# shroglck/open-pi-zero

Hardware: AMD Instinct MI355X
Metric: train samples/sec at gbsz 1024 (bf16 fwd+bwd+clip+AdamW) (higher is better)
Workload: dtype bf16; 1 GPU; Pi0 bridge training step: 256 img + 20 text + 1 proprio + 4 action tokens; model=pi0 (SigLIP-So400m/14 + Gemma-2B + 0.3B action expert), global_batch=1024, micro_batch=256, grad_accum=4, seq_len=281, parallelism=dp1

## Files before the change

### include/pz_abi.h

```cpp
#ifndef PZ_ABI_H
#define PZ_ABI_H

#include <stdint.h>

#ifdef __cplusplus
extern "C" {
#endif

#define PZ_ABI_VERSION 21

enum {
  PZ_OK = 0,
  PZ_ERR_INVALID_ARG = 1,
  PZ_ERR_LAUNCH = 2,
  PZ_ERR_UNSUPPORTED = 3,
};

enum {
  PZ_EPI_NONE = 0,
  PZ_EPI_GELU = 1,
  PZ_EPI_GEGLU = 2,
  PZ_EPI_SILU = 3,
  PZ_EPI_DGELU = 4,
  PZ_EPI_DSILU = 5,
  PZ_EPI_DGEGLU = 6,
};

typedef struct pz_gemm_args {
  int64_t M, N, K;
  const void* A; int64_t lda; int32_t a_kcontig;
  const void* B; int64_t ldb; int32_t b_kcontig;
  void* C; int64_t ldc; int32_t c_fp32;
  int64_t batch, batch_inner;
  int64_t sA_outer, sA_inner, sB_outer, sB_inner, sC_outer, sC_inner, sR_outer, sR_inner;
  int32_t epilogue;
  float alpha;
  int32_t beta_accum;
  const void* bias;
  const void* resid; int64_t ld_resid;
  void* aux; int64_t ld_aux;
  int64_t geglu_inter;
  void* workspace; int64_t ws_bytes;
  const void* norm_w; float norm_eps;
  int32_t fp8_mode; const float* a_row_scale;
} pz_gemm_args;
int pz_gemm(const pz_gemm_args* args, void* stream);
#define PZ_ABSMAX_PARTS 1024
int pz_fp8_quant_vt(const void* v, int64_t ldv, int64_t v_bstride, int64_t Z, int64_t nk, void* vt, float* vs,
                    int64_t ldt, void* stream);
int pz_fp8_quant_attn(const void* q, int64_t nqr, const void* k, int64_t nkr, const void* v, int64_t ldv,
                      int64_t v_bstride, int64_t Z, int64_t nk, void* qc, float* qs, void* kc, float* ks, void* vt,
                      float* vs, int64_t ldt, void* stream);
int pz_rmsnorm_fwd_f8(const void* x, int64_t ldx, const void* w, void* q, int64_t ldq, float* qscale, int64_t R,
                      int64_t D, float eps, void* stream);
int pz_layernorm_fwd_f8(const void* x, int64_t ldx, const void* w, const void* b, void* q, int64_t ldq, float* qscale,
                        int64_t R, int64_t D, float eps, void* stream);
int pz_fp8_quant_rows(const void* x, int64_t ldx, void* q, int64_t ldq, float* row_scale, int64_t R, int64_t D,
                      void* stream);
int pz_fp8_quant_tensor(const void* x, int64_t n, void* q, float inv_scale, void* stream);
int pz_fp8_absmax(const void* x, int64_t n, float* parts, void* stream);
const char* pz_gemm_kernel_name(const pz_gemm_args* args);

typedef struct pz_small_gemm_args {
  int64_t M, N, K;
  const void* A; int64_t sAm, sAk;
  const void* B; int64_t sBk, sBn;
  void* C; int64_t ldc;
  const void* bias;
  float alpha;
  int32_t beta;
} pz_small_gemm_args;
int pz_gemm_small(const pz_small_gemm_args* args, void* stream);

int pz_rmsnorm_fwd(const void* x, int64_t ldx, const void* w, void* y, int64_t ldy, float* rstd,
                   int64_t R, int64_t D, float eps, void* stream);
int pz_rmsnorm_bwd(const void* dy, int64_t lddy, const void* x, int64_t ldx, const void* w,
                   const float* rstd, const void* dres, void* dx, int64_t lddx, float* dw_part,
                   int64_t R, int64_t D, void* stream);
int pz_layernorm_fwd(const void* x, int64_t ldx, const void* w, const void* b, void* y, int64_t ldy,
// ... 174 lines not shown
```

### open-pi-zero_amd/csrc/pz_gemm.hip

```cpp
#include <stdarg.h>
#include <stdio.h>
#include <stdlib.h>
#include <string.h>

#include <type_traits>

#include "pz_gemm_epi.h"

namespace {

constexpr int BM = 128, BN = 128, BK = 64, NT = 256;
constexpr int TILE_BYTES = 128 * 64 * 2;


__device__ __forceinline__ i32x8 cat_f8(const bf16x8& lo, const bf16x8& hi) {
  const u32x4 a = __builtin_bit_cast(u32x4, lo), b = __builtin_bit_cast(u32x4, hi);
  return i32x8{(int)a[0], (int)a[1], (int)a[2], (int)a[3], (int)b[0], (int)b[1], (int)b[2], (int)b[3]};
}

__device__ __forceinline__ int sw_tr(int k) { return ((k & 3) | (((k >> 3) & 1) << 2)) << 2; }

template <bool KC>
__device__ __forceinline__ void g2r(u32x4 (&r)[4], const bf16_t* __restrict__ base, int64_t ld,
                                    int64_t row0, int64_t R, int64_t k0, int64_t K,
// ... 690 lines not shown
#pragma unroll
    for (int i = 0; i < CPB; ++i) {
      const int c = threadIdx.x + (half * CPB + i) * NT2;
      const int im = c >> 12, row = (c >> 4) & 255, ch = c & 15;
      const int col = im * 128 + ch * 8;
      iv[i] = *reinterpret_cast<const u32x4*>(smem + im * 65536 + row * 256 + ((ch ^ (row & 15)) << 4));
      a0[i] = X0 ? *reinterpret_cast<const u32x4*>(X0 + row * ld0 + col) : u32x4{0u, 0u, 0u, 0u};
      a1[i] = X1 ? *reinterpret_cast<const u32x4*>(X1 + row * ld1 + col) : u32x4{0u, 0u, 0u, 0u};
    }
#pragma unroll
    for (int i = 0; i < CPB; ++i) {
      const int c = threadIdx.x + (half * CPB + i) * NT2;
      const int im = c >> 12, row = (c >> 4) & 255, ch = c & 15;
      const int col = im * 128 + ch * 8;
      float v[8], x0[8], x1[8];
      unpack8(iv[i], v);
      unpack8(a0[i], x0);
      unpack8(a1[i], x1);
      bf16_t* Cp = C + row * p.ldc + col;
      if (FM == FM_DGEGLU) {
        float dg[8], du[8];
#pragma unroll
        for (int e = 0; e < 8; ++e) {
          float gl_, gr_;
          gelu_tanh_both(x0[e], gl_, gr_);
          dg[e] = v[e] * x1[e] * gr_;
          du[e] = v[e] * gl_;
        }
        st16(Cp, pack8v(dg), p.nt_store);
        st16(Cp + p.geglu_I, pack8v(du), p.nt_store);
      } else if (FM == FM_DACT) {
#pragma unroll
        for (int e = 0; e < 8; ++e) v[e] *= gelu ? gelu_tanh_grad(x0[e]) : silu_grad(x0[e]);
        st16(Cp, pack8v(v), p.nt_store);
      } else {
        if (act) {
          if (p.aux) st16(p.aux + (m0 + row) * p.ld_aux + n0 + col, iv[i], p.nt_aux);
#pragma unroll
          for (int e = 0; e < 8; ++e) v[e] = gelu ? gelu_tanh(v[e]) : silu(v[e]);
        }
#pragma unroll
        for (int e = 0; e < 8; ++e) v[e] += x1[e] + x0[e];
        st16(Cp, pack8v(v), p.nt_store);
      }
    }
  }
}

__device__ __forceinline__ void epi8p_rope(const GemmP& p, int64_t m0, int64_t n0, int wr, int wc, int lane,
                                           const f32x4 (&acc)[8][4], char* smem) {
  const int g4 = 4 * (lane >> 4), rl = lane & 15;
  char* img = smem + (wc >> 1) * 65536;
#pragma unroll
  for (int rb = 0; rb < 8; ++rb)
#pragma unroll
    for (int cb = 0; cb < 4; ++cb) {
      float v[4];
#pragma unroll
      for (int r = 0; r < 4; ++r) v[r] = acc[rb][cb][r] * p.alpha;
      img_put(img, wr * 128 + rb * 16 + rl, (wc & 1) * 64 + cb * 16 + g4, u32x2{pack2bf(v[0], v[1]), pack2bf(v[2], v[3])});
    }
  lds_sync();
  const int64_t h = n0 >> 8;
#pragma unroll 2
  for (int it = 0; it < 8; ++it) {
    const int c = threadIdx.x + it * NT2, row = c >> 4, ch = c & 15;
    const int64_t m = m0 + row;
    if (m >= p.M) continue;
    const int off = (ch ^ (row & 15)) << 4;
    const u32x4 w1 = *reinterpret_cast<const u32x4*>(smem + row * 256 + off);
    const u32x4 w2 = *reinterpret_cast<const u32x4*>(smem + 65536 + row * 256 + off);
    const int64_t b = m / p.rT, t = m - b * p.rT;
    if (h == p.rnh + 1) {
      bf16_t* dv = p.rv + (b * p.rLk + p.rkoff + t) * 256 + ch * 8;
      *reinterpret_cast<u32x4*>(dv) = w1;
      *reinterpret_cast<u32x4*>(dv + 128) = w2;
      continue;
// ... 1266 lines not shown

template <bool AKC, bool BKC, bool GEGLU, bool KTAIL>
static int launch8p_k(const GemmP& p, int64_t batch, hipStream_t st) {
  const int smem = 2 * P8_BUF;
  const bool kh = use_khalf(AKC, BKC, p.M, p.N, p.K);
  auto kern = kh ? gemm8k_kernel<AKC, BKC, GEGLU, KTAIL> : gemm8p_kernel<AKC, BKC, GEGLU, KTAIL>;
  static bool attr_set[2] = {false, false};
  if (!attr_set[kh]) {
    hipFuncSetAttribute((const void*)kern, hipFuncAttributeMaxDynamicSharedMemorySize, smem);
    attr_set[kh] = true;
  }
  const int T = p.tiles_m * p.tiles_n;
  const int units = p.tail_s ? p.dp_tiles + (T - p.dp_tiles) * p.tail_s : T;
  hipLaunchKernelGGL(kern, dim3(units, (unsigned)batch), dim3(NT2), smem, st, p);
  PZ_CHECK_LAUNCH();
  if (p.tail_s) {
    launch_tail<GEGLU>(p, T, st);
    PZ_CHECK_LAUNCH();
  }
  return PZ_OK;
}

template <bool AKC, bool BKC, bool GEGLU>
static int launch8p(const GemmP& p, int64_t batch, hipStream_t st) {
  if (p.K % 64 != 0) return launch8p_k<AKC, BKC, GEGLU, true>(p, batch, st);
  return launch8p_k<AKC, BKC, GEGLU, false>(p, batch, st);
}

static bool use_8phase() {
  const char* e = getenv("PZ_GEMM_BIG");
  return !(e && strcmp(e, "2stage") == 0);
}

extern "C" int pz_gemm(const pz_gemm_args* a, void* stream) {
  PZ_CHECK_ARG(a != nullptr, "pz_gemm: null args");
  PZ_CHECK_ARG(a->M > 0 && a->N > 0 && a->K > 0, "pz_gemm: bad dims M=%lld N=%lld K=%lld",
               (long long)a->M, (long long)a->N, (long long)a->K);
  PZ_CHECK_ARG(a->A && a->B && a->C, "pz_gemm: null operand");
  PZ_CHECK_ARG(a->batch >= 1 && a->batch_inner >= 1 && a->batch % a->batch_inner == 0,
               "pz_gemm: bad batch %lld/%lld", (long long)a->batch, (long long)a->batch_inner);
  PZ_CHECK_ARG(PZ_ALIGNED(a->A, 16) && PZ_ALIGNED(a->B, 16), "pz_gemm: A/B must be 16-byte aligned");
  PZ_CHECK_ARG(a->lda % 8 == 0 && a->ldb % 8 == 0, "pz_gemm: lda/ldb must be multiples of 8");
  PZ_CHECK_ARG(a->ldc % 4 == 0 && PZ_ALIGNED(a->C, 8), "pz_gemm: ldc %% 4 and C 8-byte alignment");
  PZ_CHECK_ARG(a->sA_outer % 8 == 0 && a->sA_inner % 8 == 0 && a->sB_outer % 8 == 0 &&
                   a->sB_inner % 8 == 0 && a->sC_outer % 4 == 0 && a->sC_inner % 4 == 0,
               "pz_gemm: batch strides must keep 16-byte alignment");
  if (a->a_kcontig) PZ_CHECK_ARG(a->K % 8 == 0, "pz_gemm: k-contiguous A needs K %% 8 == 0");
  else PZ_CHECK_ARG(a->M % 8 == 0, "pz_gemm: k-strided A needs M %% 8 == 0");
  if (a->b_kcontig) PZ_CHECK_ARG(a->K % 8 == 0, "pz_gemm: k-contiguous B needs K %% 8 == 0");
  else PZ_CHECK_ARG(a->N % 8 == 0, "pz_gemm: k-strided B needs N %% 8 == 0");
  const bool geglu = a->epilogue == PZ_EPI_GEGLU;
  if (geglu) {
    PZ_CHECK_ARG(a->b_kcontig && a->geglu_inter > 0 && a->N == 2 * a->geglu_inter && a->batch == 1 &&
                     !a->beta_accum && !a->resid && !a->bias && !a->c_fp32 && a->geglu_inter % 4 == 0,
                 "pz_gemm: GEGLU needs k-contiguous B = [gate; up] (N = 2I), no batch/bias/resid");
  }
  if (a->epilogue == PZ_EPI_GELU || a->epilogue == PZ_EPI_SILU)
    PZ_CHECK_ARG(a->batch == 1, "pz_gemm: activation epilogue is unbatched");
  PZ_CHECK_ARG(a->epilogue >= PZ_EPI_NONE && a->epilogue <= PZ_EPI_DGEGLU, "pz_gemm: unknown epilogue %d",
               (int)a->epilogue);
  PZ_CHECK_ARG(!(a->c_fp32 && a->beta_accum && a->resid), "pz_gemm: fp32 beta accumulation takes no resid");
  if (a->epilogue >= PZ_EPI_DGELU) {
    PZ_CHECK_ARG(a->batch == 1 && a->aux && !a->bias && !a->resid && !a->beta_accum && !a->c_fp32,
                 "pz_gemm: backward epilogues read aux, write bf16 C, unbatched, no bias/resid/beta");
    if (a->epilogue == PZ_EPI_DGEGLU)
      PZ_CHECK_ARG(a->geglu_inter == a->N && a->ldc >= 2 * a->N && a->ld_aux >= 2 * a->N,
// ... 25 lines not shown

  GemmP p;
  memset(&p, 0, sizeof(p));
  p.A = (const bf16_t*)a->A;
  p.B = (const bf16_t*)a->B;
  p.C = a->C;
  p.bias = (const bf16_t*)a->bias;
  p.resid = (const bf16_t*)a->resid;
  p.aux = (bf16_t*)a->aux;
  p.M = a->M; p.N = a->N; p.K = a->K;
  p.lda = a->lda; p.ldb = a->ldb; p.ldc = a->ldc;
  p.ld_resid = a->ld_resid; p.ld_aux = a->ld_aux; p.geglu_I = a->geglu_inter;
  p.batch_inner = a->batch_inner;
  p.sAo = a->sA_outer; p.sAi = a->sA_inner;
  p.sBo = a->sB_outer; p.sBi = a->sB_inner;
  p.sCo = a->sC_outer; p.sCi = a->sC_inner;
  p.sRo = a->sR_outer; p.sRi = a->sR_inner;
  p.epi = a->epilogue;
  p.c_fp32 = a->c_fp32;
  p.beta = a->beta_accum;
  p.alpha = a->alpha;
  p.nw = (const bf16_t*)a->norm_w;
  p.neps = a->norm_eps;
  p.rs = a->fp8_mode == 1 ? a->a_row_scale : nullptr;
  {
    const char* e = getenv("PZ_GEMM_DBG");
    p.dbg = e ? atoi(e) : 0;
    e = getenv("PZ_GEMM_NT");
    p.nt_store = e ? atoi(e) : 0;
    e = getenv("PZ_GEMM_NT_AUX");
    p.nt_aux = p.nt_store || (e && atoi(e) != 0);
  }
  hipStream_t st = (hipStream_t)stream;

  const Plan pl = make_plan(a);
  {
    const char* e = getenv("PZ_GEMM_GROUP");
    if (e && atoi(e) >= 1 && atoi(e) <= 64) p.group = atoi(e);
    else p.group = (a->K >= 16384 && pl.tiles_n <= 8) || a->epilogue == PZ_EPI_DGEGLU ? 2 : 8;
  }
  if (pl.kind == PATH_GEMV) return pz_gemv_launch(a, st);
  if (a->norm_w)
    PZ_CHECK_ARG((pl.kind == PATH_SKINNY || pl.kind == PATH_SKINNY64) && PZ_ALIGNED(a->norm_w, 16),
                 "pz_gemm: fused RMSNorm needs the few-row paths (M <= 64, k-contiguous A/B, K %% 32 == 0 "
                 "(M <= 16) or K %% 64 == 0) and a 16-byte aligned weight");
  if (pl.kind == PATH_SKINNY64) {
    p.tiles_n = (int)pl.tiles_n;
    if (pl.ksplit > 0) {
      p.ws = (float*)a->workspace;
      p.ksplit = pl.ksplit;
      p.ldw = pl.ldw;
      p.sk_tk = sk64_fits(pl, a) ? 0 : -1;
    }
    return pz_sk64_launch(p, pl.skinny_w, pl.skinny_nc, pl.skinny_mb, a->fp8_mode == 2, pl.tiles_n, st);
  }
  if (a->fp8_mode == 1 && pl.kind == PATH_ROWS) {
    p.tiles_m = (int)pl.tiles_m;
    p.tiles_n = (int)pl.tiles_n;
    PZ_CHECK_ARG(PZ_ALIGNED(a->A, 16) && PZ_ALIGNED(a->B, 16), "pz_gemm: W8A8 rows need 16-byte aligned codes");
    return pz_rows_launch(p, pl.rows_w, pl.rows_tnb, false, 2, st);
  }
  if (a->fp8_mode == 1) {
    p.tiles_m = (int)pl.tiles_m;
    p.tiles_n = (int)pl.tiles_n;
    PZ_CHECK_ARG(pl.tiles_m * pl.tiles_n < (1LL << 31), "pz_gemm: grid too large");
    if (pl.tail_s) {
// ... 4 lines not shown
    }
    return geglu ? launch8p_f8<true>(p, st) : launch8p_f8<false>(p, st);
  }
  if (pl.kind == PATH_SKINNY) {
    PZ_CHECK_ARG(a->batch < 65536, "pz_gemm: batch too large");
    if (pl.skinny_w == 16) return launch_skinny<16>(p, pl.skinny_nc, pl.tiles_n, a->batch, st);
    if (pl.skinny_w == 8) return launch_skinny<8>(p, pl.skinny_nc, pl.tiles_n, a->batch, st);
    return launch_skinny<4>(p, pl.skinny_nc, pl.tiles_n, a->batch, st);
  }
  p.tiles_m = (int)pl.tiles_m;
  p.tiles_n = (int)pl.tiles_n;
  PZ_CHECK_ARG(pl.tiles_m * pl.tiles_n < (1LL << 31) && a->batch < 65536, "pz_gemm: grid too large");
  if (pl.kind == PATH_ROWS)
    return pz_rows_launch(p, pl.rows_w, pl.rows_tnb, pl.geglu, pl.rows_f8, st);
  if (pl.kind == PATH_TALL) {
    if (pl.splits > 1) {
      p.ws = (float*)a->workspace;
      p.ksplit = pl.ksplit;
      p.ldw = pl.ldw;
    }
    return pz_tall_launch(p, pl.tall_mi, geglu, pl.bkc, pl.splits > 1 ? pl.splits : 1, st);
  }
  if (pl.kind == PATH_256 && use_8phase()) {
    if (pl.tail_s) {
      p.ws = (float*)a->workspace;
      p.dp_tiles = pl.dp_tiles;
      p.tail_s = pl.tail_s;
      p.tail_kt = pl.tail_kt;
    }
    if (geglu) {
      if (a->a_kcontig) return launch8p<true, true, true>(p, a->batch, st);
      return launch8p<false, true, true>(p, a->batch, st);
    }
    if (a->a_kcontig && a->b_kcontig) return launch8p<true, true, false>(p, a->batch, st);
    if (a->a_kcontig && !a->b_kcontig) return launch8p<true, false, false>(p, a->batch, st);
    if (!a->a_kcontig && a->b_kcontig) return launch8p<false, true, false>(p, a->batch, st);
    return launch8p<false, false, false>(p, a->batch, st);
  }
  if (pl.kind == PATH_256) {
    if (geglu) {
      if (a->a_kcontig) return launch256<true, true, true>(p, a->batch, st);
      return launch256<false, true, true>(p, a->batch, st);
    }
    if (a->a_kcontig && a->b_kcontig) return launch256<true, true, false>(p, a->batch, st);
    if (a->a_kcontig && !a->b_kcontig) return launch256<true, false, false>(p, a->batch, st);
    if (!a->a_kcontig && a->b_kcontig) return launch256<false, true, false>(p, a->batch, st);
    return launch256<false, false, false>(p, a->batch, st);
  }
  if (pl.kind == PATH_SPLIT) {
    p.ws = (float*)a->workspace;
    p.ksplit = pl.ksplit;
    p.ldw = pl.ldw;
  }
  if (geglu) {
    if (pl.tag) return launch_tile_any<true, true, 4, 1>(p, pl, a->batch, st);
    if (a->a_kcontig) return launch_tile_any<true, true, 4, 0>(p, pl, a->batch, st);
    return launch_tile_any<false, true, 4, 0>(p, pl, a->batch, st);
  }
  if (a->a_kcontig && a->b_kcontig) return launch_tile_any<true, true, 2, 0>(p, pl, a->batch, st);
  if (a->a_kcontig && !a->b_kcontig) return launch_tile_any<true, false, 2, 0>(p, pl, a->batch, st);
  if (!a->a_kcontig && a->b_kcontig) return launch_tile_any<false, true, 2, 0>(p, pl, a->batch, st);
  return launch_tile_any<false, false, 2, 0>(p, pl, a->batch, st);
}

extern "C" int pz_gemm_qkv_rope(const pz_qkv_rope_args* a, void* stream) {
  PZ_CHECK_ARG(a && a->x && a->W && a->pos && a->cs && a->k_out && a->v_out && a->M > 0 && a->K > 0,
               "gemm_qkv_rope: bad args");
  PZ_CHECK_ARG(a->nh >= 1 && a->N == (a->nh + 2) * a->hd && a->T > 0 && a->M % a->T == 0,
               "gemm_qkv_rope: N = (nh + 2) * hd, M %% T == 0");
  if (a->hd != BT || !a->q_out) return PZ_ERR_UNSUPPORTED;
// ... 79 lines not shown
```

### open-pi-zero_amd/csrc/pz_gemm_epi.h

```cpp
#pragma once

#include <type_traits>

#include "pz_common.h"

struct GemmP {
  const bf16_t* A;
  const bf16_t* B;
  void* C;
  const bf16_t* bias;
  const bf16_t* resid;
  bf16_t* aux;
  int64_t M, N, K, lda, ldb, ldc, ld_resid, ld_aux, geglu_I;
  int64_t batch_inner, sAo, sAi, sBo, sBi, sCo, sCi, sRo, sRi;
  int tiles_m, tiles_n, epi, c_fp32, beta;
  float alpha;
  float* ws;
  int64_t ksplit, ldw;
  int sk_tk;
  int batch_xcd;
  int dp_tiles, tail_s, tail_kt;
  const bf16_t* nw;
  float neps;
  const float* rs;
  int dbg;
  const int64_t* rpos;
  const float* rcs;
  bf16_t *rq, *rk, *rv;
  int64_t rT, rnh, rLq, rqoff, rLk, rkoff;
  int nt_store;
  int nt_aux;
  int group;
};

namespace {

__device__ __forceinline__ void tile_coords(int bid, int nwg, int tiles_m, int tiles_n, int& tm, int& tn,
                                            int GROUP = 8) {
  const int xcd = bid & 7, local = bid >> 3;
  const int q = nwg >> 3, r = nwg & 7;
  const int wg = (xcd < r ? xcd * (q + 1) : r * (q + 1) + (xcd - r) * q) + local;
  GROUP = GROUP >= 1 ? GROUP : 8;
  const int per_group = GROUP * tiles_n;
  const int g = wg / per_group;
  const int first_m = g * GROUP;
  const int gsize = min(tiles_m - first_m, GROUP);
  const int in = wg - g * per_group;
  tm = first_m + in % gsize;
  tn = in / gsize;
}

struct Side {
  u32x4 w;
};

__device__ __forceinline__ u32x2 ld4bf(const bf16_t* X, bool full, int64_t n, int64_t N) {
  if (full) return *reinterpret_cast<const u32x2*>(X);
  unsigned h[4];
#pragma unroll
  for (int r = 0; r < 4; ++r) h[r] = n + r < N ? (unsigned)X[r] : 0u;
  return u32x2{h[0] | (h[1] << 16), h[2] | (h[3] << 16)};
}
__device__ __forceinline__ void unpack4(u32x2 w, float (&o)[4]) {
  o[0] = __uint_as_float(w[0] << 16); o[1] = __uint_as_float(w[0] & 0xffff0000u);
  o[2] = __uint_as_float(w[1] << 16); o[3] = __uint_as_float(w[1] & 0xffff0000u);
// ... 135 lines not shown
  Side s;
  epi_load4<EM>(p, cofs, rofs, m, n, s);
  epi_store4<EM>(p, cofs, rofs, m, n, acc, s, epi_load_bias(p, n));
}

__device__ __forceinline__ void store_out4_rt(const GemmP& p, int64_t cofs, int64_t rofs, int64_t m, int64_t n,
                                              const f32x4& acc) {
  if (m >= p.M || n >= p.N) return;
  const bool full = n + 4 <= p.N;
  float v[4];
#pragma unroll
  for (int r = 0; r < 4; ++r) v[r] = acc[r] * p.alpha;
  if (p.epi == PZ_EPI_DGEGLU) {
    float g[4], u[4], dg[4], du[4];
    const bf16_t* X = p.aux + m * p.ld_aux + n;
    unpack4(ld4bf(X, full, n, p.N), g);
    unpack4(ld4bf(X + p.geglu_I, full, n, p.N), u);
#pragma unroll
    for (int r = 0; r < 4; ++r) {
      float gl_, gr_;
      gelu_tanh_both(g[r], gl_, gr_);
      dg[r] = v[r] * u[r] * gr_;
      du[r] = v[r] * gl_;
    }
    bf16_t* Cp = reinterpret_cast<bf16_t*>(p.C) + cofs + m * p.ldc + n;
    store4(Cp, full, n, p.N, dg);
    store4(Cp + p.geglu_I, full, n, p.N, du);
    return;
  }
  if (p.epi == PZ_EPI_DGELU || p.epi == PZ_EPI_DSILU) {
    float x[4];
    unpack4(ld4bf(p.aux + m * p.ld_aux + n, full, n, p.N), x);
#pragma unroll
    for (int r = 0; r < 4; ++r) v[r] *= p.epi == PZ_EPI_DGELU ? gelu_tanh_grad(x[r]) : silu_grad(x[r]);
  }
  if (p.bias) {
    float b[4];
    unpack4(ld4bf(p.bias + n, full, n, p.N), b);
#pragma unroll
    for (int r = 0; r < 4; ++r) v[r] += b[r];
  }
  if (p.epi == PZ_EPI_GELU || p.epi == PZ_EPI_SILU) {
    if (p.aux) store4(p.aux + m * p.ld_aux + n, full, n, p.N, v);
#pragma unroll
    for (int r = 0; r < 4; ++r) v[r] = p.epi == PZ_EPI_GELU ? gelu_tanh(v[r]) : silu(v[r]);
  }
  if (p.resid) {
    float x[4];
    unpack4(ld4bf(p.resid + rofs + m * p.ld_resid + n, full, n, p.N), x);
#pragma unroll
    for (int r = 0; r < 4; ++r) v[r] += x[r];
  }
  if (p.c_fp32) {
    float* Cp = reinterpret_cast<float*>(p.C) + cofs + m * p.ldc + n;
#pragma unroll
    for (int r = 0; r < 4; ++r)
      if (full || n + r < p.N) Cp[r] = p.beta ? Cp[r] + v[r] : v[r];
  } else {
    bf16_t* Cp = reinterpret_cast<bf16_t*>(p.C) + cofs + m * p.ldc + n;
    if (p.beta) {
      float o[4];
      unpack4(ld4bf(Cp, full, n, p.N), o);
#pragma unroll
      for (int r = 0; r < 4; ++r) v[r] += o[r];
    }
    store4(Cp, full, n, p.N, v);
  }
// ... 46 lines not shown
```

### open-pi-zero_amd/pizero_native/_lib.py

```python

from __future__ import annotations

import ctypes as C
import os

_HERE = os.path.dirname(os.path.dirname(os.path.abspath(__file__)))
LIB_PATH = os.path.join(_HERE, "libpizero_hip.so")
if os.environ.get("PZ_LIB_PATH"):
    LIB_PATH = os.path.join(_HERE, os.path.basename(os.environ["PZ_LIB_PATH"]))
    import sys as _sys

    print(f"[pizero_native] PZ_LIB_PATH override: loading {LIB_PATH} instead of the default libpizero_hip.so",
          file=_sys.stderr, flush=True)

ABI_VERSION = 21
PZ_EPI_NONE, PZ_EPI_GELU, PZ_EPI_GEGLU, PZ_EPI_SILU = 0, 1, 2, 3
PZ_EPI_DGELU, PZ_EPI_DSILU, PZ_EPI_DGEGLU = 4, 5, 6
PZ_SUMSQ_PARTS = 2048

i64, i32, f32, vp = C.c_int64, C.c_int32, C.c_float, C.c_void_p
fp = C.POINTER(C.c_float)


class GemmArgs(C.Structure):
    _fields_ = [
        ("M", i64), ("N", i64), ("K", i64),
        ("A", vp), ("lda", i64), ("a_kcontig", i32),
        ("B", vp), ("ldb", i64), ("b_kcontig", i32),
        ("C", vp), ("ldc", i64), ("c_fp32", i32),
        ("batch", i64), ("batch_inner", i64),
        ("sA_outer", i64), ("sA_inner", i64), ("sB_outer", i64), ("sB_inner", i64),
        ("sC_outer", i64), ("sC_inner", i64), ("sR_outer", i64), ("sR_inner", i64),
        ("epilogue", i32), ("alpha", f32), ("beta_accum", i32),
        ("bias", vp), ("resid", vp), ("ld_resid", i64), ("aux", vp), ("ld_aux", i64),
        ("geglu_inter", i64),
        ("workspace", vp), ("ws_bytes", i64),
        ("norm_w", vp), ("norm_eps", f32),
        ("fp8_mode", i32), ("a_row_scale", vp),
    ]


class SmallGemmArgs(C.Structure):
    _fields_ = [
        ("M", i64), ("N", i64), ("K", i64),
        ("A", vp), ("sAm", i64), ("sAk", i64),
        ("B", vp), ("sBk", i64), ("sBn", i64),
        ("C", vp), ("ldc", i64), ("bias", vp), ("alpha", f32), ("beta", i32),
    ]


class SoftmaxArgs(C.Structure):
    _fields_ = [
        ("S", vp), ("lds", i64), ("P", vp), ("ldp", i64), ("tcap", vp),
        ("R", i64), ("N", i64), ("scale", f32), ("cap", f32), ("mask_mode", i32),
        ("rows_per_batch", i64), ("heads", i64), ("qoff", i64),
        ("cnt", vp), ("prefix", i64), ("cond", i64),
        ("mask", vp), ("ldm", i64), ("mask_bstride", i64),
    ]


class FlashArgs(C.Structure):
    _fields_ = [
        ("Z", i64), ("H", i64), ("nq", i64), ("nk", i64), ("head_dim", i64),
        ("q", vp), ("ldq", i64), ("q_bstride", i64), ("q_hstride", i64),
        ("k", vp), ("ldk", i64), ("k_bstride", i64), ("k_hstride", i64),
        ("v", vp), ("ldv", i64), ("v_bstride", i64), ("v_hstride", i64),
        ("n_groups", i32),
        ("g_row0", i64 * 3), ("g_o", vp * 3), ("g_bstride", i64 * 3), ("g_ld", i64 * 3),
        ("o_hstride", i64),
        ("lse", vp),
        ("scale", f32), ("cap", f32),
# ... 20 lines not shown
class QkvRopeArgs(C.Structure):
    _fields_ = [
        ("x", vp), ("ldx", i64), ("W", vp), ("ldw", i64), ("M", i64), ("N", i64), ("K", i64),
        ("norm_w", vp), ("norm_eps", f32), ("pos", vp), ("cs", vp), ("q_out", vp), ("k_out", vp), ("v_out", vp),
        ("T", i64), ("nh", i64), ("hd", i64), ("Lq", i64), ("qoff", i64), ("Lk", i64), ("koff", i64),
        ("w_fp8", i32), ("w_scale", f32),
    ]


class ReduceSeg(C.Structure):
    _fields_ = [("part", vp), ("P", i64), ("D", i64), ("out", vp), ("beta", i32)]


class DecodeAttnArgs(C.Structure):
    _fields_ = [
        ("q", vp), ("ldq", i64), ("Lq", i64), ("qoff", i64), ("k", vp), ("v", vp), ("k_bstride", i64),
        ("v_bstride", i64), ("o", vp), ("ldo", i64), ("B", i64), ("nh", i64), ("T", i64), ("nk", i64),
        ("head_dim", i64), ("scale", f32), ("cap", f32), ("cnt", vp), ("prefix", i64), ("cond", i64),
        ("qtok0", i64), ("ws", vp), ("ws_bytes", i64),
    ]


SIGNATURES = {
    "pz_gemm": [C.POINTER(GemmArgs), vp],
    "pz_fp8_quant_rows": [vp, i64, vp, i64, vp, i64, i64, vp],
    "pz_fp8_quant_tensor": [vp, i64, vp, f32, vp],
    "pz_fp8_quant_vt": [vp, i64, i64, i64, i64, vp, vp, i64, vp],
    "pz_rmsnorm_fwd_f8": [vp, i64, vp, vp, i64, vp, i64, i64, f32, vp],
    "pz_layernorm_fwd_f8": [vp, i64, vp, vp, vp, i64, vp, i64, i64, f32, vp],
    "pz_fp8_quant_attn": [vp, i64, vp, i64, vp, i64, i64, i64, i64, vp, vp, vp, vp, vp, vp, i64, vp],
    "pz_flash_fwd_f8": [C.POINTER(FlashArgs), vp, vp, vp, vp, i64, vp, vp, i64, vp],
    "pz_fp8_absmax": [vp, i64, vp, vp],
    "pz_gemm_kernel_name": [C.POINTER(GemmArgs)],
    "pz_gemm_small": [C.POINTER(SmallGemmArgs), vp],
    "pz_rmsnorm_fwd": [vp, i64, vp, vp, i64, vp, i64, i64, f32, vp],
    "pz_rmsnorm_bwd": [vp, i64, vp, i64, vp, vp, vp, vp, i64, vp, i64, i64, vp],
    "pz_layernorm_fwd": [vp, i64, vp, vp, vp, i64, vp, vp, i64, i64, f32, vp],
    "pz_layernorm_bwd": [vp, i64, vp, i64, vp, vp, vp, vp, vp, i64, vp, vp, i64, i64, vp, vp],
    "pz_act_bwd_colsum": [vp, i64, vp, i64, vp, i64, i64, i32, vp, i64, vp, i32, vp],
    "pz_reduce_parts_multi": [vp, i32, vp],
    "pz_norm_rows_per_part": [],
    "pz_reduce_parts": [vp, i64, i64, vp, i32, vp],
    "pz_colsum": [vp, i64, i64, i64, vp, i32, vp, vp],
    "pz_batch_sum": [vp, i64, i64, i64, vp, i32, vp],
    "pz_rope_table": [vp, i64, i64, f32, vp],
    "pz_qkv_rope_split": [vp, vp, vp, vp, vp, vp, i64, i64, i64, i64, i64, i64, i64, i64, i64, vp],
    "pz_qkv_rope_split_bwd": [vp, vp, vp, vp, vp, vp, i64, i64, i64, i64, i64, i64, i64, i64, i64, vp],
    "pz_gemv_qkv_rope": [C.POINTER(QkvRopeArgs), vp],
    "pz_gemm_qkv_rope": [C.POINTER(QkvRopeArgs), vp],
    "pz_decode_attn": [C.POINTER(DecodeAttnArgs), vp],
    "pz_decode_attn_ws_bytes": [i64, i64, i64],
    "pz_attn_softmax": [C.POINTER(SoftmaxArgs), vp],
    "pz_attn_softmax_bwd": [vp, vp, i64, vp, vp, i64, i64, i64, f32, f32, vp],
    "pz_flash_fwd": [C.POINTER(FlashArgs), vp],
    "pz_flash_fwd_probs": [C.POINTER(FlashArgs), vp, vp, i64, vp],
    "pz_flash_bwd_ds": [C.POINTER(FlashArgs), vp, vp, vp, i64, vp],
    "pz_flash_bwd_prep": [C.POINTER(FlashArgs), vp],
    "pz_flash_bwd": [C.POINTER(FlashArgs), vp],
    "pz_patchify": [vp, vp, i64, i64, i64, i64, i64, vp],
    "pz_embed_merge": [vp, vp, i64, vp, vp, i64, i64, i64, i64, i64, i64, f32, f32, vp],
    "pz_embed_merge_bwd": [vp, vp, vp, i64, i64, i64, i64, i64, f32, vp],
    "pz_time_embed": [vp, vp, i64, i64, f32, i32, vp],
    "pz_concat_time": [vp, vp, vp, i64, i64, i64, vp],
    "pz_split_time_grad": [vp, vp, i64, i64, vp],
    "pz_flow_psi": [vp, vp, vp, vp, i64, i64, f32, vp],
    "pz_flow_loss": [vp, i64, i64, vp, vp, vp, vp, vp, i64, i64, i64, f32, vp],
# ... 18 lines not shown
    "pz_debug_poison_lds": [C.c_uint32, vp],
    "pz_debug_spin": [i64, i64, vp],
    "pz_last_error": [],
    "pz_abi_version": [],
}
_RESTYPE = {"pz_last_error": C.c_char_p, "pz_gemm_kernel_name": C.c_char_p, "pz_norm_rows_per_part": i64,
            "pz_decode_attn_ws_bytes": i64}

_lib = None


class NativeError(RuntimeError):
    pass


def lib():
    global _lib
    if _lib is None:
        if not os.path.exists(LIB_PATH):
            raise NativeError(
                f"{LIB_PATH} not found: build it with `python open-pi-zero_amd/build_native.py` "
                "(or __graft_entry__.build()); the Pi0 path has no CPU/eager fallback")
        L = C.CDLL(LIB_PATH)
        for name, argt in SIGNATURES.items():
            fn = getattr(L, name)
            fn.argtypes = argt
            fn.restype = _RESTYPE.get(name, C.c_int)
        if L.pz_abi_version() != ABI_VERSION:
            raise NativeError(f"{LIB_PATH}: ABI version {L.pz_abi_version()} != {ABI_VERSION}; rebuild it")
        _lib = L
    return _lib


_NO_LAUNCH = {"pz_last_error", "pz_abi_version", "pz_gemm_kernel_name", "pz_norm_rows_per_part",
              "pz_decode_attn_ws_bytes", "pz_debug_poison_lds"}
_POISON_LDS = [0xFFFFFFFF if os.environ.get("PZ_POISON_LDS", "0") == "1" else None]


_RECENT = [[] if os.environ.get("PZ_CHECK_FINITE", "0") == "1" else None]


def recent_launches(clear=True):
    r = _RECENT[0] or []
    if clear and _RECENT[0] is not None:
        _RECENT[0] = []
    return r


def set_poison_lds(word):
    _POISON_LDS[0] = None if word is None else int(word) & 0xFFFFFFFF


def call(name, *args):
    if _POISON_LDS[0] is not None and name not in _NO_LAUNCH:
        rc = lib().pz_debug_poison_lds(_POISON_LDS[0], args[-1])
        if rc != 0:
            raise NativeError(f"pz_debug_poison_lds failed (rc={rc}): {lib().pz_last_error().decode(errors='replace')}")
    if _RECENT[0] is not None:
        _RECENT[0].append(name)
    rc = getattr(lib(), name)(*args)
    if rc != 0:
        msg = lib().pz_last_error().decode(errors="replace")
        raise NativeError(f"{name} failed (rc={rc}): {msg}")
    return rc
```

### open-pi-zero_amd/pizero_native/engine.py

```python

from __future__ import annotations

import contextlib
import math
import os
import weakref
from dataclasses import dataclass

import torch

from . import ops
from .ops import PZ_EPI_DGEGLU, PZ_EPI_DGELU, PZ_EPI_GEGLU, PZ_EPI_GELU, PZ_EPI_NONE, PZ_EPI_SILU

BF16 = torch.bfloat16
F32 = torch.float32


def _cfg(cfg, key, default=None):
    from src.utils.config import cfg_get

    return cfg_get(cfg, key, default)


@dataclass
# ... 163 lines not shown
            for i, n in enumerate(w):
                if eng.rg(n):
                    ops.linear_wgrad(dm[:, i * self.D:(i + 1) * self.D], cond, eng.gw(n), beta=beta)
        if all(eng.rg(n) for n in b):
            ops.colsum(dm[:, : len(b) * self.D], eng.ar.grad_span(b[0], b[-1]), ws, beta=beta)
        else:
            for i, n in enumerate(b):
                if eng.rg(n):
                    ops.colsum(dm[:, i * self.D:(i + 1) * self.D], eng.gw(n), ws, beta=beta)


class Group:

    def __init__(self, name, prefix, mixtures, T, joint_off, hidden, inter, theta, skip_last, pos_key):
        self.name, self.prefix, self.mixtures = name, prefix, mixtures
        self.T, self.off, self.hid, self.inter, self.theta = T, joint_off, hidden, inter, theta
        self.skip_last = skip_last
        self.pos_key = pos_key


class Engine:
    def __init__(self, model):
        self.m = model
        self.d = Dims.from_cfg(model.cfg)
        self._tables = {}
        self._ws = {}
        self._jkv_holder = None
        ja = os.environ.get("PZ_JOINT_ATTN", "probs")
        self.joint_flash = ja == "flash"
        self.joint_probs = ja == "probs"
        self.joint_ds = os.environ.get("PZ_JOINT_DS", "1") == "1"
        self.joint_ds_dq = os.environ.get("PZ_JOINT_DS_DQ", "1") == "1"
        self.infer_flash = os.environ.get("PZ_INFER_ATTN", "flash") == "flash"
        self.split_dact = os.environ.get("PZ_SPLIT_DACT", "1") == "1"
        self.split_dgeglu = os.environ.get("PZ_SPLIT_DGEGLU", "0") == "1"
        self.fuse_qkv_rope = os.environ.get("PZ_FUSE_QKV_ROPE", "1") == "1" and self.d.hd == 256
        self.expert_stream = os.environ.get("PZ_EXPERT_STREAM", "1") == "1"
        self.expert_stream_fwd = os.environ.get("PZ_EXPERT_STREAM_FWD", "0") == "1"
        vI = self.d.vI
        self.sig_pitch = vI if os.environ.get("PZ_SIG_PITCH", "1") == "0" else (vI + 63) // 64 * 64
        self._side = {}
        self.check_finite = os.environ.get("PZ_CHECK_FINITE", "0") == "1"
        self.f8_attn = os.environ.get("PZ_FP8_ATTN", "1") == "1"
        self.f8 = None
        self.f8_version = None
        if self.d.nkv != 1:
            raise NotImplementedError("joint attention kernel path assumes MQA (num_key_value_heads=1, bridge.yaml:176)")

    def ada_slots(self, prefix):
        key = ("ada_slots", prefix)
        sl = self._tables.get(key)
        if sl is None:
            from src.model.vla.pizero import adaln_slots

            sl = self._tables[key] = adaln_slots(prefix, self.d.nL, self.d.ada)
        return sl

    def _chk(self, where, **tensors):
        if not self.check_finite:
            return
        check_finite(where, **tensors)

    @property
    def ar(self):
        return self.m._arena

    def w(self, name):
# ... 248 lines not shown
        fb = os.environ.get("PZ_FUSED_BIAS_GRAD", "1") != "0" and os.environ.get("PZ_NORM_BWD", "row")[:1] != "w"
        pd = torch.empty(P, d.vH, device=dev, dtype=F32) if fb else None
        pdn = torch.empty(P, d.vH, device=dev, dtype=F32) if fb else None
        pd2 = torch.empty(P, d.vH, device=dev, dtype=F32) if fb else None
        multi = os.environ.get("PZ_REDUCE_MULTI", "1") != "0"
        pw2 = torch.empty(P, d.vH, device=dev, dtype=F32) if multi else pw
        pb2 = torch.empty(P, d.vH, device=dev, dtype=F32) if multi else pb
        ws_act = self.colsum_ws_rows(1024, d.vI) if fb else None
        nm = "multi_modal_projector.linear."
        if self.rg(nm + "weight"):
            ops.linear_wgrad(dimg, sv["y"], self.gw(nm + "weight"), beta=beta)
        if self.rg(nm + "bias"):
            ops.colsum(dimg, self.gw(nm + "bias"), ws, beta=beta)
        dy = torch.empty(M, d.vH, device=dev, dtype=BF16)
        ops.linear_dgrad(dimg, self.w(nm + "weight"), dy)
        dx = torch.empty_like(dy)
        ops.layernorm_bwd(dy, sv["x_last"], self.w(vt + "post_layernorm.weight"), sv["mu"], sv["r"], dx,
                          dw_part=pw, db_part=pb, dx_part=pd)
        self._norm_grads(vt + "post_layernorm.", pw, pb, beta)
        nh, hd = d.vheads, d.vH // d.vheads
        Np = d.img_tok
        W3 = 3 * d.vH
        dg = self._sig_rows(M, dev)
        delta = torch.empty(B * nh, Np, device=dev, dtype=F32)
        dqkv = torch.empty(M, W3, device=dev, dtype=BF16)
        dh = torch.empty(M, d.vH, device=dev, dtype=BF16)
        dxm = torch.empty(M, d.vH, device=dev, dtype=BF16)
        dO = torch.empty(M, d.vH, device=dev, dtype=BF16)
        for i in reversed(range(d.vL)):
            p = f"{vt}encoder.layers.{i}."
            st = sv["layers"][i]
            red = [] if multi else None
            fc1b = self.rg(p + "mlp.fc1.bias")
            if self.split_dact:
                ops.linear_dgrad(dx, self.w(p + "mlp.fc2.weight"), dg)
                if fb and fc1b:
                    ops.act_bwd_colsum(dg, st["a1"], dg, PZ_EPI_GELU, ws_act, self.gw(p + "mlp.fc1.bias"), beta=beta)
                else:
                    ops.act_bwd(dg, st["a1"], dg, None, PZ_EPI_GELU)
            else:
                ops.linear_dgrad(dx, self.w(p + "mlp.fc2.weight"), dg, epi=PZ_EPI_DGELU, aux=st["a1"])
            if self.rg(p + "mlp.fc2.weight"):
                ops.linear_wgrad(dx, st["g1"], self.gw(p + "mlp.fc2.weight"), beta=beta)
            st["g1"] = None
            if self.rg(p + "mlp.fc2.bias"):
                if fb:
                    self._reduce(red, pd, self.gw(p + "mlp.fc2.bias"), beta)
                else:
                    ops.colsum(dx, self.gw(p + "mlp.fc2.bias"), ws, beta=beta)
            if self.rg(p + "mlp.fc1.weight"):
                ops.linear_wgrad(dg, st["h2"], self.gw(p + "mlp.fc1.weight"), beta=beta)
            if fc1b and not (fb and self.split_dact):
                ops.colsum(dg, self.gw(p + "mlp.fc1.bias"), ws, beta=beta)
            ops.linear_dgrad(dg, self.w(p + "mlp.fc1.weight"), dh)
            ops.layernorm_bwd(dh, st["xm"], self.w(p + "layer_norm2.weight"), st["mu2"], st["r2"], dxm, dres=dx,
                              dw_part=pw2, db_part=pb2, dx_part=pd2)
            self._norm_grads(p + "layer_norm2.", pw2, pb2, beta, red)
            if self.rg(p + "self_attn.out_proj.weight"):
                ops.linear_wgrad(dxm, st["O"], self.gw(p + "self_attn.out_proj.weight"), beta=beta)
            if self.rg(p + "self_attn.out_proj.bias"):
                if fb:
                    self._reduce(red, pd2, self.gw(p + "self_attn.out_proj.bias"), beta)
                else:
                    ops.colsum(dxm, self.gw(p + "self_attn.out_proj.bias"), ws, beta=beta)
            ops.linear_dgrad(dxm, self.w(p + "self_attn.out_proj.weight"), dO)
            ops.flash_bwd(ops.siglip_flash_args(st["qkv"], st["O"], st["lse"], B, nh, hd, Np, dO=dO, delta=delta,
                                                dqkv=dqkv))
            qn, vn = p + "self_attn.q_proj.", p + "self_attn.v_proj."
            if all(self.rg(p + f"self_attn.{k}_proj.weight") for k in "qkv"):
                ops.linear_wgrad(dqkv, st["h1"], self.ar.grad_span(qn + "weight", vn + "weight"), beta=beta)
            else:
                for k, c0 in (("q", 0), ("k", d.vH), ("v", 2 * d.vH)):
                    if self.rg(p + f"self_attn.{k}_proj.weight"):
                        ops.linear_wgrad(dqkv[:, c0:c0 + d.vH], st["h1"], self.gw(p + f"self_attn.{k}_proj.weight"),
                                         beta=beta)
            if all(self.rg(p + f"self_attn.{k}_proj.bias") for k in "qkv"):
                ops.colsum(dqkv, self.ar.grad_span(qn + "bias", vn + "bias"), ws, beta=beta)
            ops.linear_dgrad(dqkv, self.qkv_siglip(p), dh)
            dxn = torch.empty_like(dx)
            ops.layernorm_bwd(dh, st["x"], self.w(p + "layer_norm1.weight"), st["mu1"], st["r1"], dxn, dres=dxm,
                              dw_part=pw, db_part=pb, dx_part=pdn)
            self._norm_grads(p + "layer_norm1.", pw, pb, beta, red)
            if red:
                ops.reduce_parts_multi(red, beta=beta)
            pd, pdn = pdn, pd
# ... 1068 lines not shown
```

### open-pi-zero_amd/pizero_native/ops.py

```python

from __future__ import annotations

import ctypes as C

import torch

from ._lib import (
    PZ_EPI_DGEGLU,
    PZ_EPI_DGELU,
    PZ_EPI_DSILU,
    PZ_EPI_GEGLU,
    PZ_EPI_GELU,
    PZ_EPI_NONE,
    PZ_EPI_SILU,
    PZ_SUMSQ_PARTS,
    AdamW8Args,
    QkvRopeArgs,
    DecodeAttnArgs,
    FlashArgs,
    GemmArgs,
    SmallGemmArgs,
    NativeError,
    SoftmaxArgs,
    call,
# ... 163 lines not shown
              resid, 0 if resid is None else resid.stride(0), aux, 0 if aux is None else aux.stride(0),
              N // 2 if epi == PZ_EPI_GEGLU else 0, 1, 1, (0, 0), (0, 0), (0, 0), (0, 0), workspace(out.device),
              norm)
    a.fp8_mode = 2 if x_scale is None else 1
    a.a_row_scale = _p(x_scale)
    call("pz_gemm", C.byref(a), _st())
    return out


def rows_w8a8_ok(M, K, ncols, epi=PZ_EPI_NONE):
    import os

    if os.environ.get("PZ_ROWS_W8A8") == "0":
        return False
    return 64 < M <= 1024 and K % 128 == 0 and K <= 2048 and ncols <= 4096 and epi != PZ_EPI_GEGLU


def rows_w8a16_ok(M, K, ncols):
    import os

    if os.environ.get("PZ_GEMM_ROWS") == "0" or os.environ.get("PZ_ROWS_W8A16") == "0":
        return False
    maxm = int(os.environ.get("PZ_ROWS_MAXM", "1024"))
    return 64 < M <= maxm and K % 64 == 0 and (os.environ.get("PZ_GEMM_ROWS") == "1" or (K <= 2048 and ncols <= 4096))


def linear_dgrad(dy, W, dx, *, beta=False, resid=None, epi=PZ_EPI_NONE, aux=None):
    M, N = dy.shape
    K = W.shape[1]
    gemm(M, K, N, dy, dy.stride(0), True, W, W.stride(0), False, dx, dx.stride(0), beta=beta,
         resid=resid, ld_resid=0 if resid is None else resid.stride(0), epi=epi, aux=aux,
         ld_aux=0 if aux is None else aux.stride(0), geglu_inter=K if epi == PZ_EPI_DGEGLU else 0)
    return dx


def _split_k(M, N, K):
    tiles = ((N + 255) // 256) * ((K + 255) // 256)
    if tiles >= 160 or M < 4096 or N < 512 or K < 512 or M % 8 == 0:
        return 1
    best = 1
    for s in (2, 4, 8):
        if M % (s * 64) == 0:
            best = s
            if tiles * s >= 240:
                break
    return best


def linear_wgrad(dy, x, dW, *, beta=False):
    M, N = dy.shape
    K = x.shape[1]
    S = _split_k(M, N, K) if dW.is_contiguous() else 1
    if S == 1:
        gemm(N, K, M, dy, dy.stride(0), False, x, x.stride(0), False, dW, dW.stride(0), beta=beta)
        return dW
    Mc = M // S
    slabs = torch.empty(S, N, K, device=dW.device, dtype=torch.float32)
    gemm(N, K, Mc, dy, dy.stride(0), False, x, x.stride(0), False, slabs, K, batch=S,
         sA=(Mc * dy.stride(0), 0), sB=(Mc * x.stride(0), 0), sC=(N * K, 0))
    reduce_parts(slabs.view(S, N * K), dW.view(-1), beta=beta)
    return dW


def small_linear(x, W, out, *, bias=None, beta=False):
    M, K = x.shape
    N = W.shape[0]
# ... 418 lines not shown
```

Baseline: 272.9 samples/s.

## Fuse GELU-backward bias column-sum into the dgrad GEMM epilogue

The SigLIP MLP backward now produces fc1 bias gradient partial sums inside the fc2 dgrad GEMM's DACT epilogue. The bf16 outputs are staged through LDS and summed per row chunk into a workspace, which the existing reduce then folds into the bias gradient. An edge kernel covers leftover columns, and split_dact now defaults to off, so the separate act_bwd_colsum pass over dg is skipped when the fused path is supported. The epilogue gains an extra LDS pass and sync. The non-8-phase DACT path now rounds to bf16 before the derivative multiply, which slightly changes numerics.

```diff
diff --git a/include/pz_abi.h b/include/pz_abi.h
--- a/include/pz_abi.h
+++ b/include/pz_abi.h
@@ -7,7 +7,7 @@
 extern "C" {
 #endif
 
-#define PZ_ABI_VERSION 21
+#define PZ_ABI_VERSION 22
 
 enum {
   PZ_OK = 0,
@@ -43,8 +43,10 @@
   void* workspace; int64_t ws_bytes;
   const void* norm_w; float norm_eps;
   int32_t fp8_mode; const float* a_row_scale;
+  float* dact_colsum; int64_t dact_colsum_rows;
 } pz_gemm_args;
 int pz_gemm(const pz_gemm_args* args, void* stream);
+int pz_gemm_dact_colsum_ok(const pz_gemm_args* args);
 #define PZ_ABSMAX_PARTS 1024
 int pz_fp8_quant_vt(const void* v, int64_t ldv, int64_t v_bstride, int64_t Z, int64_t nk, void* vt, float* vs,
                     int64_t ldt, void* stream);
diff --git a/open-pi-zero_amd/csrc/pz_gemm.hip b/open-pi-zero_amd/csrc/pz_gemm.hip
--- a/open-pi-zero_amd/csrc/pz_gemm.hip
+++ b/open-pi-zero_amd/csrc/pz_gemm.hip
@@ -746,7 +746,9 @@
       } else if (FM == FM_DACT) {
 #pragma unroll
         for (int e = 0; e < 8; ++e) v[e] *= gelu ? gelu_tanh_grad(x0[e]) : silu_grad(x0[e]);
-        st16(Cp, pack8v(v), p.nt_store);
+        const u32x4 o = pack8v(v);
+        st16(Cp, o, p.nt_store);
+        if (p.csum) *reinterpret_cast<u32x4*>(smem + im * 65536 + row * 256 + ((ch ^ (row & 15)) << 4)) = o;
       } else {
         if (act) {
           if (p.aux) st16(p.aux + (m0 + row) * p.ld_aux + n0 + col, iv[i], p.nt_aux);
@@ -757,6 +759,25 @@
         for (int e = 0; e < 8; ++e) v[e] += x1[e] + x0[e];
         st16(Cp, pack8v(v), p.nt_store);
       }
+    }
+  }
+  if (FM == FM_DACT && p.csum) {
+    lds_sync();
+    const int t = threadIdx.x, rc = t >> 7, cp = t & 127;
+    if (rc * p.crpc < BT) {
+      const int im = cp >> 6, col = (cp & 63) * 2, ch = col >> 3;
+      const char* base = smem + im * 65536 + (col & 7) * 2;
+      float s0 = 0.f, s1 = 0.f;
+      for (int i = 0; i < p.crpc; i += 16) {
+#pragma unroll
+        for (int j = 0; j < 16; ++j) {
+          const unsigned w = *reinterpret_cast<const unsigned*>(base + (rc * p.crpc + i + j) * 256 + ((ch ^ j) << 4));
+          s0 += __uint_as_float(w << 16);
+          s1 += __uint_as_float(w & 0xffff0000u);
+        }
+      }
+      float* W = p.csum + (m0 / p.crpc + rc) * p.N + n0 + im * 128 + col;
+      *reinterpret_cast<float2*>(W) = float2{s0, s1};
     }
   }
 }
@@ -2089,6 +2110,45 @@
   return !(e && strcmp(e, "2stage") == 0);
 }
 
+static int64_t dact_colsum_rpc(const pz_gemm_args* a) {
+  if (!a || !a->dact_colsum || a->dact_colsum_rows <= 0 || a->M <= 0 || a->M % BT != 0) return 0;
+  if (a->epilogue != PZ_EPI_DGELU && a->epilogue != PZ_EPI_DSILU) return 0;
+  if (a->batch != 1 || a->fp8_mode != 0 || a->c_fp32 || a->N % 8 != 0 || a->ldc % 8 != 0 || !PZ_ALIGNED(a->C, 16) ||
+      !PZ_ALIGNED(a->dact_colsum, 16))
+    return 0;
+  int64_t chunks = a->dact_colsum_rows < (a->M + 15) / 16 ? a->dact_colsum_rows : (a->M + 15) / 16;
+  const int64_t rpc = (a->M + chunks - 1) / chunks;
+  if (rpc != 64 && rpc != 128 && rpc != 256) return 0;
+  if (!use_8phase()) return 0;
+  const Plan pl = make_plan(a);
+  return pl.kind == PATH_256 && pl.tail_s == 0 ? rpc : 0;
+}
+
+extern "C" int pz_gemm_dact_colsum_ok(const pz_gemm_args* a) { return dact_colsum_rpc(a) != 0; }
+
+__global__ void __launch_bounds__(64) dact_colsum_edge_kernel(const bf16_t* __restrict__ X, int64_t ld, int64_t c0,
+                                                              int64_t N, int64_t rpc, float* ws) {
+  const int64_t c = c0 + threadIdx.x * 8;
+  if (c >= N) return;
+  const bf16_t* x = X + (int64_t)blockIdx.x * rpc * ld + c;
+  float s[8] = {0.f, 0.f, 0.f, 0.f, 0.f, 0.f, 0.f, 0.f};
+  for (int64_t r = 0; r < rpc; r += 8) {
+    u32x4 w[8];
+#pragma unroll
+    for (int u = 0; u < 8; ++u) w[u] = *reinterpret_cast<const u32x4*>(x + (r + u) * ld);
+#pragma unroll
+    for (int u = 0; u < 8; ++u) {
+      float v[8];
+      unpack8(w[u], v);
+#pragma unroll
+      for (int e = 0; e < 8; ++e) s[e] += v[e];
+    }
+  }
+  float* W = ws + (int64_t)blockIdx.x * N + c;
+  *reinterpret_cast<f32x4*>(W) = f32x4{s[0], s[1], s[2], s[3]};
+  *reinterpret_cast<f32x4*>(W + 4) = f32x4{s[4], s[5], s[6], s[7]};
+}
+
 extern "C" int pz_gemm(const pz_gemm_args* a, void* stream) {
   PZ_CHECK_ARG(a != nullptr, "pz_gemm: null args");
   PZ_CHECK_ARG(a->M > 0 && a->N > 0 && a->K > 0, "pz_gemm: bad dims M=%lld N=%lld K=%lld",
@@ -2180,6 +2240,12 @@
     p.nt_aux = p.nt_store || (e && atoi(e) != 0);
   }
   hipStream_t st = (hipStream_t)stream;
+  if (a->dact_colsum) {
+    const int64_t rpc = dact_colsum_rpc(a);
+    if (!rpc) return PZ_ERR_UNSUPPORTED;
+    p.csum = a->dact_colsum;
+    p.crpc = (int)rpc;
+  }
 
   const Plan pl = make_plan(a);
   {
@@ -2250,10 +2316,17 @@
       if (a->a_kcontig) return launch8p<true, true, true>(p, a->batch, st);
       return launch8p<false, true, true>(p, a->batch, st);
     }
-    if (a->a_kcontig && a->b_kcontig) return launch8p<true, true, false>(p, a->batch, st);
-    if (a->a_kcontig && !a->b_kcontig) return launch8p<true, false, false>(p, a->batch, st);
-    if (!a->a_kcontig && a->b_kcontig) return launch8p<false, true, false>(p, a->batch, st);
-    return launch8p<false, false, false>(p, a->batch, st);
+    int rc;
+    if (a->a_kcontig && a->b_kcontig) rc = launch8p<true, true, false>(p, a->batch, st);
+    else if (a->a_kcontig && !a->b_kcontig) rc = launch8p<true, false, false>(p, a->batch, st);
+    else if (!a->a_kcontig && a->b_kcontig) rc = launch8p<false, true, false>(p, a->batch, st);
+    else rc = launch8p<false, false, false>(p, a->batch, st);
+    if (rc == PZ_OK && p.csum && a->N % BT != 0) {
+      hipLaunchKernelGGL(dact_colsum_edge_kernel, dim3((unsigned)(a->M / p.crpc)), dim3(64), 0, st,
+                         (const bf16_t*)a->C, a->ldc, a->N / BT * BT, a->N, (int64_t)p.crpc, p.csum);
+      PZ_CHECK_LAUNCH();
+    }
+    return rc;
   }
   if (pl.kind == PATH_256) {
     if (geglu) {
diff --git a/open-pi-zero_amd/csrc/pz_gemm_epi.h b/open-pi-zero_amd/csrc/pz_gemm_epi.h
--- a/open-pi-zero_amd/csrc/pz_gemm_epi.h
+++ b/open-pi-zero_amd/csrc/pz_gemm_epi.h
@@ -31,6 +31,8 @@
   int nt_store;
   int nt_aux;
   int group;
+  float* csum;
+  int crpc;
 };
 
 namespace {
@@ -232,7 +234,8 @@
     float x[4];
     unpack4(ld4bf(p.aux + m * p.ld_aux + n, full, n, p.N), x);
 #pragma unroll
-    for (int r = 0; r < 4; ++r) v[r] *= p.epi == PZ_EPI_DGELU ? gelu_tanh_grad(x[r]) : silu_grad(x[r]);
+    for (int r = 0; r < 4; ++r)
+      v[r] = bf2f(f2bf(v[r])) * (p.epi == PZ_EPI_DGELU ? gelu_tanh_grad(x[r]) : silu_grad(x[r]));
   }
   if (p.bias) {
     float b[4];
diff --git a/open-pi-zero_amd/pizero_native/_lib.py b/open-pi-zero_amd/pizero_native/_lib.py
--- a/open-pi-zero_amd/pizero_native/_lib.py
+++ b/open-pi-zero_amd/pizero_native/_lib.py
@@ -13,7 +13,7 @@
     print(f"[pizero_native] PZ_LIB_PATH override: loading {LIB_PATH} instead of the default libpizero_hip.so",
           file=_sys.stderr, flush=True)
 
-ABI_VERSION = 21
+ABI_VERSION = 22
 PZ_EPI_NONE, PZ_EPI_GELU, PZ_EPI_GEGLU, PZ_EPI_SILU = 0, 1, 2, 3
 PZ_EPI_DGELU, PZ_EPI_DSILU, PZ_EPI_DGEGLU = 4, 5, 6
 PZ_SUMSQ_PARTS = 2048
@@ -37,6 +37,7 @@
         ("workspace", vp), ("ws_bytes", i64),
         ("norm_w", vp), ("norm_eps", f32),
         ("fp8_mode", i32), ("a_row_scale", vp),
+        ("dact_colsum", vp), ("dact_colsum_rows", i64),
     ]
 
 
@@ -123,6 +124,7 @@
     "pz_flash_fwd_f8": [C.POINTER(FlashArgs), vp, vp, vp, vp, i64, vp, vp, i64, vp],
     "pz_fp8_absmax": [vp, i64, vp, vp],
     "pz_gemm_kernel_name": [C.POINTER(GemmArgs)],
+    "pz_gemm_dact_colsum_ok": [C.POINTER(GemmArgs)],
     "pz_gemm_small": [C.POINTER(SmallGemmArgs), vp],
     "pz_rmsnorm_fwd": [vp, i64, vp, vp, i64, vp, i64, i64, f32, vp],
     "pz_rmsnorm_bwd": [vp, i64, vp, i64, vp, vp, vp, vp, i64, vp, i64, i64, vp],
@@ -207,7 +209,7 @@
     return _lib
 
 
-_NO_LAUNCH = {"pz_last_error", "pz_abi_version", "pz_gemm_kernel_name", "pz_norm_rows_per_part",
+_NO_LAUNCH = {"pz_last_error", "pz_abi_version", "pz_gemm_kernel_name", "pz_gemm_dact_colsum_ok", "pz_norm_rows_per_part",
               "pz_decode_attn_ws_bytes", "pz_debug_poison_lds"}
 _POISON_LDS = [0xFFFFFFFF if os.environ.get("PZ_POISON_LDS", "0") == "1" else None]
 
diff --git a/open-pi-zero_amd/pizero_native/engine.py b/open-pi-zero_amd/pizero_native/engine.py
--- a/open-pi-zero_amd/pizero_native/engine.py
+++ b/open-pi-zero_amd/pizero_native/engine.py
@@ -219,7 +219,7 @@
         self.joint_ds = os.environ.get("PZ_JOINT_DS", "1") == "1"
         self.joint_ds_dq = os.environ.get("PZ_JOINT_DS_DQ", "1") == "1"
         self.infer_flash = os.environ.get("PZ_INFER_ATTN", "flash") == "flash"
-        self.split_dact = os.environ.get("PZ_SPLIT_DACT", "1") == "1"
+        self.split_dact = os.environ.get("PZ_SPLIT_DACT", "0") == "1"
         self.split_dgeglu = os.environ.get("PZ_SPLIT_DGEGLU", "0") == "1"
         self.fuse_qkv_rope = os.environ.get("PZ_FUSE_QKV_ROPE", "1") == "1" and self.d.hd == 256
         self.expert_stream = os.environ.get("PZ_EXPERT_STREAM", "1") == "1"
@@ -534,7 +534,12 @@
             st = sv["layers"][i]
             red = [] if multi else None
             fc1b = self.rg(p + "mlp.fc1.bias")
-            if self.split_dact:
+            rows = 0
+            if not self.split_dact and fb and fc1b:
+                rows = ops.linear_dgrad_colsum(dx, self.w(p + "mlp.fc2.weight"), dg, PZ_EPI_DGELU, st["a1"], ws_act)
+            if rows:
+                self._reduce(red, ws_act[:rows], self.gw(p + "mlp.fc1.bias"), beta)
+            elif self.split_dact or (fb and fc1b):
                 ops.linear_dgrad(dx, self.w(p + "mlp.fc2.weight"), dg)
                 if fb and fc1b:
                     ops.act_bwd_colsum(dg, st["a1"], dg, PZ_EPI_GELU, ws_act, self.gw(p + "mlp.fc1.bias"), beta=beta)
@@ -552,7 +557,7 @@
                     ops.colsum(dx, self.gw(p + "mlp.fc2.bias"), ws, beta=beta)
             if self.rg(p + "mlp.fc1.weight"):
                 ops.linear_wgrad(dg, st["h2"], self.gw(p + "mlp.fc1.weight"), beta=beta)
-            if fc1b and not (fb and self.split_dact):
+            if fc1b and not fb:
                 ops.colsum(dg, self.gw(p + "mlp.fc1.bias"), ws, beta=beta)
             ops.linear_dgrad(dg, self.w(p + "mlp.fc1.weight"), dh)
             ops.layernorm_bwd(dh, st["xm"], self.w(p + "layer_norm2.weight"), st["mu2"], st["r2"], dxm, dres=dx,
diff --git a/open-pi-zero_amd/pizero_native/ops.py b/open-pi-zero_amd/pizero_native/ops.py
--- a/open-pi-zero_amd/pizero_native/ops.py
+++ b/open-pi-zero_amd/pizero_native/ops.py
@@ -219,6 +219,19 @@
          resid=resid, ld_resid=0 if resid is None else resid.stride(0), epi=epi, aux=aux,
          ld_aux=0 if aux is None else aux.stride(0), geglu_inter=K if epi == PZ_EPI_DGEGLU else 0)
     return dx
+
+
+def linear_dgrad_colsum(dy, W, dx, epi, aux, ws):
+    M, N = dy.shape
+    K = W.shape[1]
+    a = _args(M, K, N, dy, dy.stride(0), True, W, W.stride(0), False, dx, dx.stride(0), epi, 1.0, False, None, None, 0,
+              aux, aux.stride(0), 0, 1, 1, (0, 0), (0, 0), (0, 0), (0, 0), workspace(dx.device))
+    a.dact_colsum, a.dact_colsum_rows = _p(ws), ws.numel() // K
+    if not lib().pz_gemm_dact_colsum_ok(C.byref(a)):
+        return 0
+    call("pz_gemm", C.byref(a), _st())
+    chunks = min(ws.numel() // K, (M + 15) // 16)
+    return M // ((M + chunks - 1) // chunks)
 
 
 def _split_k(M, N, K):
```

Measured after the change: 274.0 samples/s (median of 6 runs). No clear change (+0.4%).
